# yahoo/TensorFlowOnSpark

Hardware: AMD Instinct MI355X
Metric: images/sec (whole node) ResNet-50 sync-SGD InputMode.SPARK (higher is better)
Workload: dtype bf16; 1 GPU; model=resnet50, global_batch=1024, per_gpu_batch=1024, parallelism=dp1

## Files before the change

### csrc/bindings.cpp

```cpp
#include <torch/extension.h>
#include <c10/hip/HIPStream.h>
#include <hip/hip_runtime.h>

extern "C" {
int tfosr_bn_fast_blocks(long, int, int, int);
void tfosr_bn_stats(const void*, int, int, float*, int, int, int, long, hipStream_t);
void tfosr_bn_finalize(const float*, int, const void*, int, int, long,
                       float*, float*, float*, float*,
                       long, int, float, float, hipStream_t);
void tfosr_bn_apply(const void*, const void*, void*, unsigned char*,
                    const float*, const float*,
                    const float*, const float*, int, int, int, long, int, long,
                    hipStream_t);
void tfosr_bn_bwd_stats(const void*, const void*, const void*,
                        const unsigned char*, void*,
                        const float*, const float*, float*, int, int, int,
                        int, int, int, long, hipStream_t);
void tfosr_bn_bwd_merge(const float*, int, float*, float*, int, hipStream_t);
void tfosr_bn_bwd_dx(const void*, const void*, const void*,
                     const unsigned char*, const float*,
                     const float*, const float*, const float*, const float*,
                     void*, int, int, int, long, int, long, hipStream_t);
int tfosr_xent_dense_grid(int, int, long, long, int, int);
void tfosr_xent_dense_fwd(int, const void*, const long*, float*, float*, float*,
                          int*, int, long, long, int, long, float, int,
                          hipStream_t);
void tfosr_xent_dense_finalize(const float*, const int*, int, int, float*, int*,
                               hipStream_t);
void tfosr_xent_dense_bwd(int, const void*, const float*, const long*,
                          const float*, const float*, const int*, int, void*,
                          int, long, long, int, long, float, int, hipStream_t);
void tfosr_nhwc_pack(const void*, void*, const float*, const float*, float, int,
                     int, long, int, long, hipStream_t);
void tfosr_sgd_step(float*, const float*, float*, float, float, float, int, long,
                    hipStream_t);
void tfosr_adam_step(float*, const float*, float*, float*, float, float, float,
                     float, float, int, int, long, hipStream_t);
void tfosr_gemm_bt(const void*, const void*, void*, int, int, int, int,
                   hipStream_t);
void tfosr_gemm_bt_acc(const void*, const void*, void*, int, int, int, int,
                       int, hipStream_t);
void tfosr_mfma_probe(const short*, const short*, float*, hipStream_t);
void tfosr_maxpool_fwd(const void*, void*, unsigned char*, int, int, int, int,
                       int, int, int, int, int, int, hipStream_t);
void tfosr_maxpool_bwd(const void*, const unsigned char*, void*, int, int, int,
                       int, int, int, int, int, int, int, hipStream_t);
void tfosr_conv3x3(const void*, const void*, const void*, void*, int, int, int,
                   int, int, int, int, int, int, int, hipStream_t);
void tfosr_conv_mfma(const void*, const void*, const void*, void*, int, int,
                     int, int, int, int, int, int, int, int, int, int, int,
                     int, int, hipStream_t);
void tfosr_conv_wrw(const void*, const void*, float*, int, int, int, int, int,
                    int, int, int, int, int, hipStream_t);
int tfosr_wrw2_split(int, int, long);
void tfosr_conv_wrw2(const void*, const void*, const void*, float*, float*,
                     int, int, int, int, int, int, int, int, int, int, int,
                     int, int, hipStream_t);
void tfosr_conv_stem(const void*, const void*, const void*, void*, int, int,
// ... 152 lines not shown
  int bf = dtype_flag(x);
  bn_check_like(dy, x, l.nhwc, false, "dy");
  bn_check_like(y, x, l.nhwc, true, "y");
  bn_check_channel_vec(w, x, l.C, "weight");
  bn_check_channel_vec(save_mean, x, l.C, "save_mean");
  bn_check_channel_vec(save_rstd, x, l.C, "save_rstd");
  dy = l.nhwc ? dy.contiguous(at::MemoryFormat::ChannelsLast) : dy.contiguous();
  auto opts = x.options().dtype(at::kFloat);
  long total = (long)l.N * l.HW * l.C;
  int nb = tfosr_bn_fast_blocks(total, l.C, bf, l.nhwc);
  auto ws = nb > 0 ? at::empty({(long)nb * 2 * l.C}, opts)
                   : at::zeros({2L * l.C}, opts);
  auto dg = at::empty({l.C}, opts);
  auto db = at::empty({l.C}, opts);
  auto dx = at::empty_like(x);
  at::Tensor gout;
  void* gout_ptr = nullptr;
  if (grad_res) {
    gout = at::empty_like(x);
    gout_ptr = gout.data_ptr();
  }
  auto s = cur_stream();
  const unsigned char* mask_ptr =
      mask.numel() ? mask.data_ptr<unsigned char>() : nullptr;
  TORCH_CHECK(!(relu && nb > 0) || mask_ptr != nullptr,
              "fast-path relu backward requires the forward bitmask");
  if (relu && nb > 0) {
    TORCH_CHECK(mask.device() == x.device() && mask.scalar_type() == at::kByte &&
                    mask.is_contiguous() && mask.numel() == total / (bf ? 8 : 4),
                "bn: mask must be the contiguous uint8 bitmask bn_fwd_train "
                "returned for this input");
  }
  tfosr_bn_bwd_stats(x.data_ptr(), dy.data_ptr(), y.data_ptr(), mask_ptr,
                     gout_ptr,
                     save_mean.data_ptr<float>(), save_rstd.data_ptr<float>(),
                     ws.data_ptr<float>(), nb, bf, l.nhwc,
                     relu, l.N, l.C, l.HW, s);
  tfosr_bn_bwd_merge(ws.data_ptr<float>(), nb, dg.data_ptr<float>(),
                     db.data_ptr<float>(), l.C, s);
  if (grad_res) {
    tfosr_bn_bwd_dx(x.data_ptr(), gout.data_ptr(), y.data_ptr(), nullptr,
                    save_mean.data_ptr<float>(), save_rstd.data_ptr<float>(),
                    w.data_ptr<float>(), dg.data_ptr<float>(), db.data_ptr<float>(),
                    dx.data_ptr(), bf, l.nhwc, 0, total, l.C, l.HW, s);
    return {dx, dg, db, gout};
  }
  tfosr_bn_bwd_dx(x.data_ptr(), dy.data_ptr(), y.data_ptr(), mask_ptr,
                  save_mean.data_ptr<float>(), save_rstd.data_ptr<float>(),
                  w.data_ptr<float>(), dg.data_ptr<float>(), db.data_ptr<float>(),
                  dx.data_ptr(), bf, l.nhwc, relu, total, l.C, l.HW, s);
  return {dx, dg, db};
}


enum { XENT_ROWS = 0, XENT_STRIDED = 1, XENT_TILE = 2 };
enum { XENT_NONE = 0, XENT_SUM = 1, XENT_MEAN = 2 };

struct XentLayout {
  int family;
  long P, S;
  int C;
};

XentLayout xent_layout(const at::Tensor& logits, const at::Tensor& target) {
  TORCH_CHECK(logits.is_cuda(), "xent: logits must be a GPU tensor");
  TORCH_CHECK(logits.scalar_type() == at::kFloat ||
                  logits.scalar_type() == at::kBFloat16,
              "xent: logits must be float32 or bfloat16");
  TORCH_CHECK(logits.dim() >= 2, "xent: logits must be (P, C) or (N, C, d1, ...)");
  TORCH_CHECK(target.device() == logits.device(),
              "xent: target must be on ", logits.device());
  TORCH_CHECK(target.scalar_type() == at::kLong, "xent: target must be int64");
  TORCH_CHECK(target.is_contiguous(), "xent: target must be contiguous");
  TORCH_CHECK(target.dim() == logits.dim() - 1 &&
                  target.size(0) == logits.size(0),
              "xent: target must have the logits' shape without the class dim");
  for (int64_t d = 2; d < logits.dim(); ++d)
    TORCH_CHECK(target.size(d - 1) == logits.size(d),
                "xent: target must have the logits' shape without the class dim");
  TORCH_CHECK(logits.size(1) >= 1 && logits.size(1) < (1L << 24),
              "xent: bad class count");
  XentLayout l;
  l.C = (int)logits.size(1);
  l.P = target.numel();
  l.S = 1;
  bool rows;
  if (logits.dim() == 2) {
    TORCH_CHECK(logits.is_contiguous(), "xent: 2-D logits must be contiguous");
    rows = true;
  } else if (logits.is_contiguous()) {
    rows = false;
    for (int64_t d = 2; d < logits.dim(); ++d) l.S *= logits.size(d);
  } else {
    TORCH_CHECK(logits.dim() == 4 &&
                    logits.is_contiguous(at::MemoryFormat::ChannelsLast),
                "xent: N-D logits must be contiguous or 4-D channels_last");
    rows = true;
  }
  l.family = rows ? (l.C >= 64 ? XENT_ROWS : XENT_TILE) : XENT_STRIDED;
  return l;
}

void xent_check_rowvec(const at::Tensor& t, const at::Tensor& logits, long P,
                       const char* name) {
  TORCH_CHECK(t.device() == logits.device() && t.scalar_type() == at::kFloat &&
                  t.is_contiguous() && t.numel() == P,
// ... 136 lines not shown
  TORCH_CHECK(p.scalar_type() == at::kFloat, "sgd_step expects fp32 params");
  tfosr_sgd_step(p.data_ptr<float>(), g.data_ptr<float>(), m.data_ptr<float>(),
                 (float)lr, (float)mu, (float)wd, nesterov, p.numel(),
                 cur_stream());
}

at::Tensor gemm_bt(at::Tensor a, at::Tensor b, bool out_bf16) {
  TORCH_CHECK(a.dim() == 2 && b.dim() == 2 && a.size(1) == b.size(1),
              "gemm_bt: A[M,K], B[N,K]");
  TORCH_CHECK(a.scalar_type() == at::kBFloat16 && b.scalar_type() == at::kBFloat16);
  int M = a.size(0), N = b.size(0), K = a.size(1);
  if (K % 32 != 0) {
    int Kp = (K + 31) / 32 * 32;
    auto ap = at::zeros({M, Kp}, a.options());
    auto bp = at::zeros({N, Kp}, b.options());
    ap.narrow(1, 0, K).copy_(a);
    bp.narrow(1, 0, K).copy_(b);
    a = ap; b = bp; K = Kp;
  }
  a = a.contiguous();
  b = b.contiguous();
  auto out = at::empty({M, N}, a.options().dtype(out_bf16 ? at::kBFloat16
                                                          : at::kFloat));
  tfosr_gemm_bt(a.data_ptr(), b.data_ptr(), out.data_ptr(), out_bf16, M, N, K,
                cur_stream());
  return out;
}

at::Tensor gemm_bf16(at::Tensor a, at::Tensor b) {
  return gemm_bt(a, b.t().contiguous(), false);
}

at::Tensor mfma_probe(at::Tensor a, at::Tensor b) {
  TORCH_CHECK(a.sizes() == at::IntArrayRef({64, 8}) &&
              b.sizes() == at::IntArrayRef({64, 8}));
  auto c = at::empty({64, 4}, a.options().dtype(at::kFloat));
  tfosr_mfma_probe(a.contiguous().data_ptr<short>(),
                   b.contiguous().data_ptr<short>(), c.data_ptr<float>(),
                   cur_stream());
  return c;
}

}

#define TFOSR_API_VERSION 6

static constexpr long kMaxTapReach = 1L << 20;

PYBIND11_MODULE(TORCH_EXTENSION_NAME, m) {
  m.def("api_version", []() { return TFOSR_API_VERSION; });
  m.def("bn_fwd_train", &bn_fwd_train);
  m.def("bn_fwd_eval", &bn_fwd_eval);
  m.def("bn_bwd", &bn_bwd);
  m.def("softmax_xent_fwd", &softmax_xent_fwd);
  m.def("softmax_xent_bwd", &softmax_xent_bwd);
  m.def("xent_dense_fwd", &xent_dense_fwd, py::arg("logits"), py::arg("target"),
        py::arg("ignore_index") = -100, py::arg("label_smoothing") = 0.0,
        py::arg("reduction") = 0, py::arg("max_grid") = 0);
  m.def("xent_dense_bwd", &xent_dense_bwd, py::arg("logits"), py::arg("lse"),
        py::arg("target"), py::arg("gout"), py::arg("nvalid") = py::none(),
        py::arg("ignore_index") = -100, py::arg("label_smoothing") = 0.0,
        py::arg("reduction") = 0, py::arg("max_grid") = 0);
  m.def("nhwc_pack", &nhwc_pack);
  m.def("sgd_step", &sgd_step);
  m.def("adam_step", [](at::Tensor p, at::Tensor g, at::Tensor m, at::Tensor v,
                        double lr, double b1, double b2, double eps, double wd,
                        long step, bool decoupled) {
    TORCH_CHECK(p.scalar_type() == at::kFloat);
    tfosr_adam_step(p.data_ptr<float>(), g.data_ptr<float>(),
                    m.data_ptr<float>(), v.data_ptr<float>(), lr, b1, b2, eps,
                    wd, (int)step, decoupled, p.numel(), cur_stream());
  });
  m.def("gemm_bt", &gemm_bt, py::arg("a"), py::arg("b"), py::arg("out_bf16") = false);
  m.def("gemm_bf16", &gemm_bf16);
  m.def("mfma_probe", &mfma_probe);
  m.def("maxpool_fwd", [](at::Tensor x, long K, long S, long P) {
    TORCH_CHECK(x.dim() == 4 && x.is_contiguous(at::MemoryFormat::ChannelsLast),
                "maxpool_fwd expects channels_last");
    int N = x.size(0), C = x.size(1), H = x.size(2), W = x.size(3);
    int OH = (H + 2 * P - K) / S + 1, OW = (W + 2 * P - K) / S + 1;
    TORCH_CHECK(C % (x.scalar_type() == at::kBFloat16 ? 8 : 4) == 0);
    auto y = at::empty({N, C, OH, OW}, x.options(),
                       at::MemoryFormat::ChannelsLast);
    auto idx = at::empty({N, OH, OW, C}, x.options().dtype(at::kByte));
    tfosr_maxpool_fwd(x.data_ptr(), y.data_ptr(), idx.data_ptr<unsigned char>(),
                      x.scalar_type() == at::kBFloat16, N, C, H, W, OH, OW,
                      K, S, P, cur_stream());
    return std::vector<at::Tensor>{y, idx};
  });
  m.def("conv3x3_fwd", [](at::Tensor x, at::Tensor w9, long Cout, long S,
                          long P) {
    TORCH_CHECK(x.dim() == 4 && x.is_contiguous(at::MemoryFormat::ChannelsLast),
                "conv3x3_fwd expects channels_last input");
    TORCH_CHECK(x.scalar_type() == at::kBFloat16 &&
                w9.scalar_type() == at::kBFloat16);
    int N = x.size(0), Cin = x.size(1), H = x.size(2), W = x.size(3);
    TORCH_CHECK(Cin % 32 == 0, "conv3x3 requires Cin % 32 == 0");
    TORCH_CHECK(w9.size(1) == 9 * Cin);
    int OH = (H + 2 * P - 3) / S + 1, OW = (W + 2 * P - 3) / S + 1;
    auto y = at::empty({N, Cout, OH, OW}, x.options(),
                       at::MemoryFormat::ChannelsLast);
    auto guard = at::zeros({64}, x.options());
    tfosr_conv3x3(x.data_ptr(), w9.contiguous().data_ptr(), guard.data_ptr(),
                  y.data_ptr(), 1, N, H, W, Cin, Cout, OH, OW,
                  S, P, cur_stream());
    return y;
// ... 230 lines not shown
```

### csrc/bn_relu.hip

```cpp
#include "tfosr_common.h"

typedef unsigned int u32;


template <typename T>
struct VecIO;

template <>
struct VecIO<bf16_t> {
  static constexpr int V = 8;
  using vec_t = s8v;
  __device__ static void load(const bf16_t* p, float* out) {
    vec_t v = *(const vec_t*)p;
    #pragma unroll
    for (int j = 0; j < 8; ++j) {
      union { short s; bf16_t b; } u;
      u.s = v[j];
      out[j] = (float)u.b;
    }
  }
  __device__ static void store(bf16_t* p, const float* in) {
    vec_t v;
    #pragma unroll
    for (int j = 0; j < 8; ++j) {
// ... 183 lines not shown
}

__global__ void bwd_stats_merge(const float* __restrict__ partials, int nblocks,
                                u32 C, float* __restrict__ dg,
                                float* __restrict__ db) {
  __shared__ float scratch[8];
  const u32 c = blockIdx.x;
  float sg = 0.f, sb = 0.f;
  for (int b = threadIdx.x; b < nblocks; b += blockDim.x) {
    sg += partials[(size_t)b * 2 * C + c];
    sb += partials[(size_t)b * 2 * C + C + c];
  }
  sg = block_sum<256>(sg, scratch);
  __syncthreads();
  sb = block_sum<256>(sb, scratch);
  if (threadIdx.x == 0) {
    dg[c] = sg;
    db[c] = sb;
  }
}

template <typename T, bool RELU>
__global__ void bwd_dx_fast(const T* __restrict__ x, const T* __restrict__ dy,
                            const unsigned char* __restrict__ mask,
                            T* __restrict__ dx,
                            const float* __restrict__ mean,
                            const float* __restrict__ rstd,
                            const float* __restrict__ w,
                            const float* __restrict__ dg,
                            const float* __restrict__ db,
                            u32 nvec, u32 C, float invM) {
  constexpr int V = VecIO<T>::V;
  const u32 c0 = channel_slot<V>(C);
  float sc[V], mu[V], rs[V], dgm[V], dbm[V], xv[V], dv[V];
  #pragma unroll
  for (int j = 0; j < V; ++j) {
    mu[j] = mean[c0 + j]; rs[j] = rstd[c0 + j];
    sc[j] = w[c0 + j] * rs[j];
    dgm[j] = dg[c0 + j] * invM;
    dbm[j] = db[c0 + j] * invM;
  }
  const u32 stride = gridDim.x * blockDim.x;
  for (u32 i = blockIdx.x * blockDim.x + threadIdx.x; i < nvec; i += stride) {
    VecIO<T>::load(x + (size_t)i * V, xv);
    VecIO<T>::load(dy + (size_t)i * V, dv);
    unsigned char m = RELU ? mask[i] : 0;
    #pragma unroll
    for (int j = 0; j < V; ++j) {
      float g = RELU ? (((m >> j) & 1) ? dv[j] : 0.f) : dv[j];
      float xhat = (xv[j] - mu[j]) * rs[j];
      dv[j] = sc[j] * (g - dbm[j] - xhat * dgm[j]);
    }
    VecIO<T>::store(dx + (size_t)i * V, dv);
  }
}


#define TFOSR_BN_CHUNK 4096

template <bool NHWC>
__device__ __forceinline__ long pixel_index(long m, int c, int C, long HW) {
  return NHWC ? m * C + c : ((m / HW) * C + c) * HW + m % HW;
}

static inline dim3 generic_red_grid(long M, int C) {
  long chunks = (M + TFOSR_BN_CHUNK - 1) / TFOSR_BN_CHUNK;
  if (chunks > 1024) chunks = 1024;
  return dim3((unsigned)C, (unsigned)(chunks > 0 ? chunks : 1));
}

template <typename T, bool NHWC>
__global__ void stats_generic(const T* __restrict__ x, float* __restrict__ ws,
                              long M, int C, long HW) {
  __shared__ float scratch[8];
  __shared__ float shift;
  const int c = blockIdx.x;
  if (threadIdx.x == 0)
    shift = channel_shift(x, c, C, HW, NHWC,
                          M < TFOSR_BN_SHIFT_PIXELS ? (int)M : TFOSR_BN_SHIFT_PIXELS);
  __syncthreads();
  const float k = shift;
  float s = 0.f, q = 0.f;
  for (long m0 = (long)blockIdx.y * TFOSR_BN_CHUNK; m0 < M;
       m0 += (long)gridDim.y * TFOSR_BN_CHUNK) {
    const long m1 = m0 + TFOSR_BN_CHUNK < M ? m0 + TFOSR_BN_CHUNK : M;
    for (long m = m0 + threadIdx.x; m < m1; m += blockDim.x) {
      float d = (float)x[pixel_index<NHWC>(m, c, C, HW)] - k;
      s += d;
      q += d * d;
    }
  }
  s = block_sum<256>(s, scratch);
  __syncthreads();
  q = block_sum<256>(q, scratch);
  if (threadIdx.x == 0) {
    atomicAdd(&ws[c], s);
    atomicAdd(&ws[C + c], q);
  }
}

template <typename T, bool NHWC, bool RELU, bool ADD>
__global__ void bn_apply_generic(const T* __restrict__ x, const T* __restrict__ res,
                                 T* __restrict__ y,
                                 const float* __restrict__ mean,
                                 const float* __restrict__ rstd,
                                 const float* __restrict__ w,
// ... 208 lines not shown
                   else { if (wg) BS_GEN(bf16_t, true, false, true); else BS_GEN(bf16_t, true, false, false); } }
    else { if (relu) { if (wg) BS_GEN(bf16_t, false, true, true); else BS_GEN(bf16_t, false, true, false); }
           else { if (wg) BS_GEN(bf16_t, false, false, true); else BS_GEN(bf16_t, false, false, false); } }
  } else {
    if (is_nhwc) { if (relu) { if (wg) BS_GEN(float, true, true, true); else BS_GEN(float, true, true, false); }
                   else { if (wg) BS_GEN(float, true, false, true); else BS_GEN(float, true, false, false); } }
    else { if (relu) { if (wg) BS_GEN(float, false, true, true); else BS_GEN(float, false, true, false); }
           else { if (wg) BS_GEN(float, false, false, true); else BS_GEN(float, false, false, false); } }
  }
#undef BS_GEN
}

void tfosr_bn_bwd_merge(const float* partials, int nb, float* dg, float* db,
                        int C, hipStream_t s) {
  hipLaunchKernelGGL(bwd_stats_merge, dim3(C), dim3(256), 0, s,
                     partials, nb > 0 ? nb : 1, (u32)C, dg, db);
}

void tfosr_bn_bwd_dx(const void* x, const void* dy, const void* y,
                     const unsigned char* mask,
                     const float* mean, const float* rstd, const float* w,
                     const float* dg, const float* db, void* dx, int is_bf16,
                     int is_nhwc, int relu, long total, int C, long HW,
                     hipStream_t s) {
  const float invM = 1.f / (float)(total / C);
  int vec = is_bf16 ? 8 : 4;
  if (fast_ok(is_nhwc, total, C, vec)) {
    u32 nvec = (u32)(total / vec);
    int grid = fast_grid(nvec, grid_quantum(C, vec));
#define DX_FAST(T, R) \
    hipLaunchKernelGGL((bwd_dx_fast<T, R>), dim3(grid), dim3(256), 0, s, \
                       (const T*)x, (const T*)dy, mask, (T*)dx, \
                       mean, rstd, w, dg, db, nvec, (u32)C, invM)
    if (is_bf16) { if (relu) DX_FAST(bf16_t, true); else DX_FAST(bf16_t, false); }
    else { if (relu) DX_FAST(float, true); else DX_FAST(float, false); }
#undef DX_FAST
    return;
  }
  int grid = tfosr_grid(total, 256);
#define DX_GEN(T, L, R) \
  hipLaunchKernelGGL((bwd_dx_generic<T, L, R>), dim3(grid), dim3(256), 0, s, \
                     (const T*)x, (const T*)dy, (const T*)y, (T*)dx, \
                     mean, rstd, w, dg, db, total, C, HW, invM)
  if (is_bf16) {
    if (is_nhwc) { if (relu) DX_GEN(bf16_t, true, true); else DX_GEN(bf16_t, true, false); }
    else { if (relu) DX_GEN(bf16_t, false, true); else DX_GEN(bf16_t, false, false); }
  } else {
    if (is_nhwc) { if (relu) DX_GEN(float, true, true); else DX_GEN(float, true, false); }
    else { if (relu) DX_GEN(float, false, true); else DX_GEN(float, false, false); }
  }
#undef DX_GEN
}

}
```

### tensorflowonspark_amd/ops/modules.py

```python

import torch
import torch.nn as nn
import torch.nn.functional as F

from . import get_ext




def _use_wrw2(k, cin, cout):
    import os
    mode = os.environ.get("TFOS_WRW", "auto")
    if mode == "mfma2":
        return True
    if mode in ("miopen", "mfma"):
        return False
    return k == 3 and cin <= 64 and cout <= 64



class _FusedBNFn(torch.autograd.Function):

    @staticmethod
    def forward(ctx, x, res, weight, bias, running_mean, running_var,
# ... 888 lines not shown
            bc1 = 1 - self.b1 ** self.step_count
            bc2 = 1 - self.b2 ** self.step_count
            upd = (m / bc1) / ((v / bc2).sqrt() + self.eps)
            if self.decoupled and self.weight_decay:
                upd = upd + self.weight_decay * pf
            pf.add_(upd, alpha=-self.lr)

    def zero_grad(self):
        self.engine.zero_grad()



class _BottleneckFn(torch.autograd.Function):

    @staticmethod
    def forward(ctx, x, w1, g1, b1, rm1, rv1, w2, g2, b2, rm2, rv2,
                w3, g3, b3, rm3, rv3, wd, gd, bd, rmd, rvd,
                stride, momentum, eps, packs=None):
        ext = get_ext(required=True)
        N, Cin, H, W = x.shape
        C1, C2, C3 = w1.shape[0], w2.shape[0], w3.shape[0]

        def as2d(t):
            return t.permute(0, 2, 3, 1).reshape(-1, t.shape[1])

        def as4d(t2, h, w):
            return t2.view(N, h, w, -1).permute(0, 3, 1, 2)

        if packs is not None:
            w1b = packs["w1b"].reshape(C1, Cin)
            w9 = packs["w9"].reshape(C2, 9 * C1)
            w3b = packs["w3b"].reshape(C3, C2)
        else:
            w1b = w1.view(C1, Cin).to(torch.bfloat16).contiguous()
            w9 = w2.permute(0, 2, 3, 1).reshape(C2, 9 * C1) \
                .to(torch.bfloat16).contiguous()
            w3b = w3.view(C3, C2).to(torch.bfloat16).contiguous()
        t1 = as4d(ext.gemm_bt(as2d(x), w1b, True), H, W)
        a1, m1, r1, k1 = ext.bn_fwd_train(t1, None, g1, b1, rm1, rv1,
                                          momentum, eps, True)
        t2 = ext.conv_mfma(a1, w9, C2, 3, 3, stride, 1, 1, -1, -1)
        a2, m2, r2, k2 = ext.bn_fwd_train(t2, None, g2, b2, rm2, rv2,
                                          momentum, eps, True)
        OH, OW = t2.shape[2], t2.shape[3]
        t3 = as4d(ext.gemm_bt(as2d(a2), w3b, True), OH, OW)

        if wd is not None:
            wdb = packs["wdb"].reshape(C3, Cin) if packs is not None \
                else wd.view(C3, Cin).to(torch.bfloat16).contiguous()
            if stride == 1:
                td = as4d(ext.gemm_bt(as2d(x), wdb, True), H, W)
            else:
                td = ext.conv_mfma(x, wdb, C3, 1, 1, stride, 0, 1, -1, -1)
            idn, md, rd, _kd = ext.bn_fwd_train(td, None, gd, bd, rmd, rvd,
                                                momentum, eps, False)
            opt = [td, idn, md, rd]
        else:
            idn = None
            opt = []
        res = idn if idn is not None else x
        y, m3, r3, k3 = ext.bn_fwd_train(t3, res, g3, b3, rm3, rv3,
                                         momentum, eps, True)

        ctx.save_for_backward(x, w1, g1, t1, a1, m1, r1, k1,
                              w2, g2, t2, a2, m2, r2, k2,
                              w3, g3, t3, m3, r3, k3, y, wd, gd, *opt)
        ctx.meta = (stride, wd is not None)
        ctx.packs = packs
        return y

    @staticmethod
    def backward(ctx, dy):
        ext = get_ext(required=True)
        (x, w1, g1, t1, a1, m1, r1, k1, w2, g2, t2, a2, m2, r2, k2,
         w3, g3, t3, m3, r3, k3, y, wd, gd, *opt) = ctx.saved_tensors
        stride, has_down = ctx.meta
        packs = ctx.packs
        N, Cin, H, W = x.shape
        C1, C2, C3 = w1.shape[0], w2.shape[0], w3.shape[0]
        OH, OW = t2.shape[2], t2.shape[3]
        dy = dy.contiguous(memory_format=torch.channels_last)
        if dy.dtype != torch.bfloat16:
            dy = dy.to(torch.bfloat16)

        def as2d(t):
            return t.permute(0, 2, 3, 1).reshape(-1, t.shape[1])

        def as4d(t2d, h, w):
            return t2d.view(N, h, w, -1).permute(0, 3, 1, 2)

        def cl(t):
            return t.contiguous(memory_format=torch.channels_last)

        dt3, dg3, db3, dres = ext.bn_bwd(t3, dy, y, k3, g3, m3, r3,
                                         True, True)
        dt3 = cl(dt3)

        def lib_wrw(dyt, xt, w4, s_, p_):
            w4 = w4.to(torch.bfloat16).contiguous(
                memory_format=torch.channels_last)
            _, dw, _ = torch.ops.aten.convolution_backward(
                dyt, xt, w4, None, [s_, s_], [p_, p_], [1, 1], False, [0, 0],
                1, [False, True, False])
            return dw

        w3bT = packs["w3bT"].reshape(C2, C3) if packs is not None \
            else w3.view(C3, C2).to(torch.bfloat16).t().contiguous()
        da2 = cl(as4d(ext.gemm_bt(as2d(dt3), w3bT, True), OH, OW))
        dw3 = ext.conv_wrw2(dt3, a2, 1, 1, 1, 0).view(C3, C2, 1, 1) \
            if _use_wrw2(1, C2, C3) \
            else lib_wrw(dt3, a2, w3.view(C3, C2, 1, 1), 1, 0)

        dt2, dg2, db2 = ext.bn_bwd(t2, da2, a2, k2, g2, m2, r2, True, False)
        dt2 = cl(dt2)

        if stride == 2:
            da1 = torch.empty(N, C1, H, W, device=x.device,
                              dtype=torch.bfloat16) \
                .contiguous(memory_format=torch.channels_last)
            if packs is not None:
                _conv_parity_packed(dt2, packs, "w9p", da1, 3, 1)
            else:
                wperm2 = w2.flip(2, 3).permute(1, 2, 3, 0) \
                    .to(torch.bfloat16).contiguous()
                _conv_parity(dt2, wperm2, da1, 3, 1)
        else:
            w9p = packs["w9p"].reshape(C1, 9 * C2) if packs is not None \
                else w2.flip(2, 3).permute(1, 2, 3, 0).reshape(C1, 9 * C2) \
                .to(torch.bfloat16).contiguous()
            da1 = ext.conv_mfma(dt2, w9p, C1, 3, 3, 1, 1, 1, H, W)
        if _use_wrw2(3, C1, C2):
            dw9 = ext.conv_wrw2(dt2, a1, 3, 3, stride, 1)
            dw2 = dw9.view(C2, 3, 3, C1).permute(0, 3, 1, 2).contiguous()
        else:
            dw2 = lib_wrw(dt2, a1, w2, stride, 1)

        dt1, dg1, db1 = ext.bn_bwd(t1, da1, a1, k1, g1, m1, r1, True, False)
        dt1 = cl(dt1)

        dw1 = ext.conv_wrw2(dt1, x, 1, 1, 1, 0).view(C1, Cin, 1, 1) \
            if _use_wrw2(1, Cin, C1) \
            else lib_wrw(dt1, x, w1.view(C1, Cin, 1, 1), 1, 0)

        w1bT = packs["w1bT"].reshape(Cin, C1) if packs is not None \
            else w1.view(C1, Cin).to(torch.bfloat16).t().contiguous()
        if has_down:
            td, idn, md, rd = opt
            dtd, dgd, dbd = ext.bn_bwd(td, dres, idn,
                                       torch.empty(0, dtype=torch.uint8,
                                                   device=td.device),
                                       gd, md, rd, False, False)
            dtd = cl(dtd)
            dwd = ext.conv_wrw2(dtd, x, 1, 1, stride, 0) \
                .view(C3, Cin, 1, 1) if _use_wrw2(1, Cin, C3) \
                else lib_wrw(dtd, x, wd.view(C3, Cin, 1, 1), stride, 0)
            dx2d = ext.gemm_bt(as2d(dt1), w1bT, True)
            dx = cl(as4d(dx2d, H, W))
            wdbT = packs["wdbT"].reshape(Cin, C3) if packs is not None \
                else wd.view(C3, Cin).to(torch.bfloat16).t().contiguous()
            if stride == 1:
                ext.gemm_bt_acc(as2d(dtd), wdbT, as2d(dx))
            else:
                ext.conv_par(dtd, wdbT, dx, [0], [0], 0, True)
            dwd = dwd.to(wd.dtype)
            dgd_, dbd_ = dgd, dbd
        else:
            dx = dres
            ext.gemm_bt_acc(as2d(dt1), w1bT, as2d(dx))
            dwd = dgd_ = dbd_ = None

        return (dx, dw1.to(w1.dtype), dg1, db1, None, None,
                dw2.to(w2.dtype), dg2, db2, None, None,
                dw3.to(w3.dtype), dg3, db3, None, None,
                dwd, dgd_, dbd_, None, None,
                None, None, None, None)



class _StemConvFn(torch.autograd.Function):

    @staticmethod
    def forward(ctx, x, weight, w224=None):
        ext = get_ext(required=True)
        N, _, H, W = x.shape
        Cout = weight.shape[0]
        x4 = torch.zeros(N, 4, H + 6, W + 6, dtype=torch.bfloat16,
                         device=x.device) \
            .contiguous(memory_format=torch.channels_last)
        x4[:, :3, 3:H + 3, 3:W + 3] = x
        if w224 is None:
            w224 = torch.zeros(Cout, 7, 8, 4, dtype=torch.bfloat16,
                               device=x.device)
            w224[:, :, :7, :3] = weight.permute(0, 2, 3, 1).to(torch.bfloat16)
        y = ext.conv_stem(x4, w224.reshape(Cout, 224).contiguous(), Cout)
        ctx.save_for_backward(x4, weight)
        return y

    @staticmethod
    def backward(ctx, dy):
        ext = get_ext(required=True)
        x4, weight = ctx.saved_tensors
        dy = dy.contiguous(memory_format=torch.channels_last)
        if dy.dtype != torch.bfloat16:
            dy = dy.to(torch.bfloat16)
# ... 101 lines not shown
```

Baseline: 9818 images/sec.

## Fuse downsample and main-branch BatchNorm into dual BN kernels for bottleneck blocks

For bottleneck blocks with a downsample branch, the two BatchNorms (bn3 and the downsample bn) are computed jointly. One apply kernel normalises both inputs, adds them, applies ReLU and writes the mask. In backward, a single stats pass and a single dx pass produce gradients for both branches. This avoids materialising the normalised identity tensor and cuts several full-tensor read/write passes and kernel launches. The cost is more live registers per thread in the dual kernels, and it adds an environment-variable switch plus a new bn_stage binding.

```diff
diff --git a/csrc/bindings.cpp b/csrc/bindings.cpp
--- a/csrc/bindings.cpp
+++ b/csrc/bindings.cpp
@@ -4,6 +4,21 @@
 
 extern "C" {
 int tfosr_bn_fast_blocks(long, int, int, int);
+void tfosr_bn_apply_dual(const void*, const void*, void*, unsigned char*,
+                         const float*, const float*, const float*, const float*,
+                         const float*, const float*, const float*, const float*,
+                         int, long, int, hipStream_t);
+void tfosr_bn_bwd_stats_dual(const void*, const void*, const void*,
+                             const unsigned char*, const float*, const float*,
+                             const float*, const float*, float*, int, int, long,
+                             int, hipStream_t);
+void tfosr_bn_bwd_merge_dual(const float*, int, float*, float*, float*, float*,
+                             int, hipStream_t);
+void tfosr_bn_bwd_dx_dual(const void*, const void*, const void*,
+                          const unsigned char*, void*, void*, const float*,
+                          const float*, const float*, const float*, const float*,
+                          const float*, const float*, const float*, const float*,
+                          int, long, int, hipStream_t);
 void tfosr_bn_stats(const void*, int, int, float*, int, int, int, long, hipStream_t);
 void tfosr_bn_finalize(const float*, int, const void*, int, int, long,
                        float*, float*, float*, float*,
@@ -262,6 +277,157 @@
   return {dx, dg, db};
 }
 
+bool bn_dual_eligible(const at::Tensor& xa, const at::Tensor& xb) {
+  if (!xa.is_cuda() || !xb.is_cuda() || xa.dim() != 4) return false;
+  if (xa.scalar_type() != at::kBFloat16 && xa.scalar_type() != at::kFloat)
+    return false;
+  if (xb.scalar_type() != xa.scalar_type() || xb.device() != xa.device() ||
+      xb.sizes() != xa.sizes())
+    return false;
+  if (!xa.is_contiguous(at::MemoryFormat::ChannelsLast) ||
+      !xb.is_contiguous(at::MemoryFormat::ChannelsLast))
+    return false;
+  return tfosr_bn_fast_blocks(xa.numel(), (int)xa.size(1),
+                              xa.scalar_type() == at::kBFloat16, 1) > 0;
+}
+
+std::vector<at::Tensor> bn_dual_fwd_train(
+    at::Tensor xa, at::Tensor xb, at::Tensor w_a, at::Tensor b_a,
+    at::Tensor rm_a, at::Tensor rv_a, at::Tensor w_b, at::Tensor b_b,
+    at::Tensor rm_b, at::Tensor rv_b, double momentum, double eps) {
+  TORCH_CHECK(bn_dual_eligible(xa, xb),
+              "bn_dual: needs two same-shape channels_last GPU tensors on the "
+              "NHWC fast path");
+  auto l = bn_layout(xa);
+  int bf = dtype_flag(xa);
+  const at::Tensor* vecs[] = {&w_a, &b_a, &rm_a, &rv_a, &w_b, &b_b, &rm_b, &rv_b};
+  for (auto* t : vecs) bn_check_channel_vec(*t, xa, l.C, "per-channel vector");
+  auto opts = xa.options().dtype(at::kFloat);
+  long M = (long)l.N * l.HW;
+  long total = M * l.C;
+  int nb = tfosr_bn_fast_blocks(total, l.C, bf, 1);
+  auto ws = at::empty({(long)nb * 2 * l.C}, opts);
+  auto mean_a = at::empty({l.C}, opts), rstd_a = at::empty({l.C}, opts);
+  auto mean_b = at::empty({l.C}, opts), rstd_b = at::empty({l.C}, opts);
+  auto y = at::empty_like(xa);
+  auto mask = at::empty({total / (bf ? 8 : 4)}, xa.options().dtype(at::kByte));
+  auto s = cur_stream();
+  auto f = [](at::Tensor& t) { return t.data_ptr<float>(); };
+  tfosr_bn_stats(xa.data_ptr(), bf, 1, f(ws), nb, l.N, l.C, l.HW, s);
+  tfosr_bn_finalize(f(ws), nb, xa.data_ptr(), bf, 1, l.HW, f(mean_a), f(rstd_a),
+                    f(rm_a), f(rv_a), M, l.C, (float)momentum, (float)eps, s);
+  tfosr_bn_stats(xb.data_ptr(), bf, 1, f(ws), nb, l.N, l.C, l.HW, s);
+  tfosr_bn_finalize(f(ws), nb, xb.data_ptr(), bf, 1, l.HW, f(mean_b), f(rstd_b),
+                    f(rm_b), f(rv_b), M, l.C, (float)momentum, (float)eps, s);
+  tfosr_bn_apply_dual(xa.data_ptr(), xb.data_ptr(), y.data_ptr(),
+                      mask.data_ptr<unsigned char>(), f(mean_a), f(rstd_a),
+                      f(w_a), f(b_a), f(mean_b), f(rstd_b), f(w_b), f(b_b), bf,
+                      total, l.C, s);
+  return {y, mean_a, rstd_a, mean_b, rstd_b, mask};
+}
+
+std::vector<at::Tensor> bn_dual_bwd(at::Tensor xa, at::Tensor xb, at::Tensor dy,
+                                    at::Tensor mask, at::Tensor w_a,
+                                    at::Tensor mean_a, at::Tensor rstd_a,
+                                    at::Tensor w_b, at::Tensor mean_b,
+                                    at::Tensor rstd_b) {
+  TORCH_CHECK(bn_dual_eligible(xa, xb),
+              "bn_dual: needs two same-shape channels_last GPU tensors on the "
+              "NHWC fast path");
+  auto l = bn_layout(xa);
+  int bf = dtype_flag(xa);
+  bn_check_like(dy, xa, true, false, "dy");
+  dy = dy.contiguous(at::MemoryFormat::ChannelsLast);
+  const at::Tensor* vecs[] = {&w_a, &mean_a, &rstd_a, &w_b, &mean_b, &rstd_b};
+  for (auto* t : vecs) bn_check_channel_vec(*t, xa, l.C, "per-channel vector");
+  long total = (long)l.N * l.HW * l.C;
+  TORCH_CHECK(mask.device() == xa.device() && mask.scalar_type() == at::kByte &&
+                  mask.is_contiguous() && mask.numel() == total / (bf ? 8 : 4),
+              "bn_dual: mask must be the contiguous uint8 bitmask "
+              "bn_dual_fwd_train returned for these inputs");
+  auto opts = xa.options().dtype(at::kFloat);
+  int nb = tfosr_bn_fast_blocks(total, l.C, bf, 1);
+  auto ws = at::empty({(long)nb * 3 * l.C}, opts);
+  auto dg_a = at::empty({l.C}, opts), dg_b = at::empty({l.C}, opts);
+  auto db_a = at::empty({l.C}, opts), db_b = at::empty({l.C}, opts);
+  auto dxa = at::empty_like(xa), dxb = at::empty_like(xb);
+  auto s = cur_stream();
+  auto f = [](at::Tensor& t) { return t.data_ptr<float>(); };
+  const unsigned char* mask_ptr = mask.data_ptr<unsigned char>();
+  tfosr_bn_bwd_stats_dual(xa.data_ptr(), xb.data_ptr(), dy.data_ptr(), mask_ptr,
+                          f(mean_a), f(rstd_a), f(mean_b), f(rstd_b), f(ws), nb,
+                          bf, total, l.C, s);
+  tfosr_bn_bwd_merge_dual(f(ws), nb, f(dg_a), f(dg_b), f(db_a), f(db_b), l.C, s);
+  tfosr_bn_bwd_dx_dual(xa.data_ptr(), xb.data_ptr(), dy.data_ptr(), mask_ptr,
+                       dxa.data_ptr(), dxb.data_ptr(), f(mean_a), f(rstd_a),
+                       f(w_a), f(dg_a), f(mean_b), f(rstd_b), f(w_b), f(dg_b),
+                       f(db_a), bf, total, l.C, s);
+  return {dxa, dxb, dg_a, dg_b, db_a, db_b};
+}
+
+void bn_stage(int family, at::Tensor x, c10::optional<at::Tensor> other,
+              c10::optional<at::Tensor> out, c10::optional<at::Tensor> mask,
+              at::Tensor ws, std::vector<at::Tensor> p, bool relu) {
+  auto l = bn_layout(x);
+  int bf = dtype_flag(x);
+  long total = (long)l.N * l.HW * l.C;
+  int nb = tfosr_bn_fast_blocks(total, l.C, bf, l.nhwc);
+  TORCH_CHECK(nb > 0, "bn_stage: shape is not on the NHWC fast path");
+  const size_t need[4] = {0, 4, 2, 5};
+  TORCH_CHECK(family >= 0 && family < 4, "bn_stage: family must be 0..3");
+  TORCH_CHECK(p.size() == need[family], "bn_stage: family ", family, " takes ",
+              need[family], " per-channel vectors");
+  for (auto& t : p) bn_check_channel_vec(t, x, l.C, "per-channel vector");
+  TORCH_CHECK(ws.device() == x.device() && ws.scalar_type() == at::kFloat &&
+                  ws.is_contiguous() && ws.numel() >= (long)nb * 2 * l.C,
+              "bn_stage: ws must hold bn_fast_blocks() * 2C floats");
+  const void* other_ptr = nullptr;
+  if (other.has_value()) {
+    bn_check_like(*other, x, l.nhwc, true, "other");
+    other_ptr = other->data_ptr();
+  }
+  void* out_ptr = nullptr;
+  if (out.has_value()) {
+    bn_check_like(*out, x, l.nhwc, true, "out");
+    out_ptr = out->data_ptr();
+  }
+  unsigned char* mask_ptr = nullptr;
+  if (mask.has_value()) {
+    TORCH_CHECK(mask->device() == x.device() && mask->scalar_type() == at::kByte &&
+                    mask->is_contiguous() && mask->numel() == total / (bf ? 8 : 4),
+                "bn_stage: mask must be a contiguous uint8 tensor, one byte "
+                "per 16 B vector");
+    mask_ptr = mask->data_ptr<unsigned char>();
+  }
+  if (family != 0 && family != 1)
+    TORCH_CHECK(other_ptr != nullptr, "bn_stage: dy is required");
+  if (family == 1 || family == 3)
+    TORCH_CHECK(out_ptr != nullptr, "bn_stage: out is required");
+  if (family >= 2)
+    TORCH_CHECK(!relu || mask_ptr != nullptr, "bn_stage: relu needs the mask");
+  auto f = [&](size_t i) { return p[i].data_ptr<float>(); };
+  auto s = cur_stream();
+  switch (family) {
+    case 0:
+      tfosr_bn_stats(x.data_ptr(), bf, 1, ws.data_ptr<float>(), nb, l.N, l.C,
+                     l.HW, s);
+      break;
+    case 1:
+      tfosr_bn_apply(x.data_ptr(), other_ptr, out_ptr, mask_ptr, f(0), f(1),
+                     f(2), f(3), bf, 1, relu, total, l.C, l.HW, s);
+      break;
+    case 2:
+      tfosr_bn_bwd_stats(x.data_ptr(), other_ptr, nullptr, mask_ptr, out_ptr,
+                         f(0), f(1), ws.data_ptr<float>(), nb, bf, 1, relu,
+                         l.N, l.C, l.HW, s);
+      break;
+    default:
+      tfosr_bn_bwd_dx(x.data_ptr(), other_ptr, nullptr, mask_ptr, f(0), f(1),
+                      f(2), f(3), f(4), out_ptr, bf, 1, relu, total, l.C, l.HW,
+                      s);
+  }
+}
+
 
 enum { XENT_ROWS = 0, XENT_STRIDED = 1, XENT_TILE = 2 };
 enum { XENT_NONE = 0, XENT_SUM = 1, XENT_MEAN = 2 };
@@ -504,6 +670,13 @@
   m.def("bn_fwd_train", &bn_fwd_train);
   m.def("bn_fwd_eval", &bn_fwd_eval);
   m.def("bn_bwd", &bn_bwd);
+  m.def("bn_dual_eligible", &bn_dual_eligible);
+  m.def("bn_dual_fwd_train", &bn_dual_fwd_train);
+  m.def("bn_dual_bwd", &bn_dual_bwd);
+  m.def("bn_fast_blocks", [](long total, int C, bool bf16, bool nhwc) {
+    return tfosr_bn_fast_blocks(total, C, bf16, nhwc);
+  });
+  m.def("bn_stage", &bn_stage);
   m.def("softmax_xent_fwd", &softmax_xent_fwd);
   m.def("softmax_xent_bwd", &softmax_xent_bwd);
   m.def("xent_dense_fwd", &xent_dense_fwd, py::arg("logits"), py::arg("target"),
diff --git a/csrc/bn_relu.hip b/csrc/bn_relu.hip
--- a/csrc/bn_relu.hip
+++ b/csrc/bn_relu.hip
@@ -259,6 +259,174 @@
       dv[j] = sc[j] * (g - dbm[j] - xhat * dgm[j]);
     }
     VecIO<T>::store(dx + (size_t)i * V, dv);
+  }
+}
+
+
+template <typename T>
+__global__ void bn_apply_dual_fast(const T* __restrict__ xa,
+                                   const T* __restrict__ xb, T* __restrict__ y,
+                                   unsigned char* __restrict__ mask,
+                                   const float* __restrict__ mean_a,
+                                   const float* __restrict__ rstd_a,
+                                   const float* __restrict__ w_a,
+                                   const float* __restrict__ b_a,
+                                   const float* __restrict__ mean_b,
+                                   const float* __restrict__ rstd_b,
+                                   const float* __restrict__ w_b,
+                                   const float* __restrict__ b_b,
+                                   u32 nvec, u32 C) {
+  constexpr int V = VecIO<T>::V;
+  const u32 c0 = channel_slot<V>(C);
+  float sca[V], mua[V], sha[V], scb[V], mub[V], shb[V], va[V], vb[V];
+  #pragma unroll
+  for (int j = 0; j < V; ++j) {
+    sca[j] = w_a[c0 + j] * rstd_a[c0 + j];
+    mua[j] = mean_a[c0 + j];
+    sha[j] = b_a[c0 + j];
+    scb[j] = w_b[c0 + j] * rstd_b[c0 + j];
+    mub[j] = mean_b[c0 + j];
+    shb[j] = b_b[c0 + j];
+  }
+  const u32 stride = gridDim.x * blockDim.x;
+  for (u32 i = blockIdx.x * blockDim.x + threadIdx.x; i < nvec; i += stride) {
+    VecIO<T>::load(xa + (size_t)i * V, va);
+    VecIO<T>::load(xb + (size_t)i * V, vb);
+    unsigned char m = 0;
+    #pragma unroll
+    for (int j = 0; j < V; ++j) {
+      float o = (va[j] - mua[j]) * sca[j] + sha[j];
+      o += (vb[j] - mub[j]) * scb[j] + shb[j];
+      if (o > 0.f) m |= (1u << j);
+      va[j] = fmaxf(o, 0.f);
+    }
+    VecIO<T>::store(y + (size_t)i * V, va);
+    mask[i] = m;
+  }
+}
+
+template <typename T>
+__global__ void bwd_stats_dual_fast(const T* __restrict__ xa,
+                                    const T* __restrict__ xb,
+                                    const T* __restrict__ dy,
+                                    const unsigned char* __restrict__ mask,
+                                    const float* __restrict__ mean_a,
+                                    const float* __restrict__ rstd_a,
+                                    const float* __restrict__ mean_b,
+                                    const float* __restrict__ rstd_b,
+                                    float* __restrict__ partials, u32 nvec,
+                                    u32 C) {
+  extern __shared__ float lds[];
+  constexpr int V = VecIO<T>::V;
+  const u32 c0 = channel_slot<V>(C);
+  for (u32 i = threadIdx.x; i < 3 * C; i += blockDim.x) lds[i] = 0.f;
+  __syncthreads();
+  float sga[V], sgb[V], sb[V], av[V], bv[V], dv[V];
+  float mua[V], rsa[V], mub[V], rsb[V];
+  #pragma unroll
+  for (int j = 0; j < V; ++j) {
+    sga[j] = 0.f; sgb[j] = 0.f; sb[j] = 0.f;
+    mua[j] = mean_a[c0 + j]; rsa[j] = rstd_a[c0 + j];
+    mub[j] = mean_b[c0 + j]; rsb[j] = rstd_b[c0 + j];
+  }
+  const u32 stride = gridDim.x * blockDim.x;
+  for (u32 i = blockIdx.x * blockDim.x + threadIdx.x; i < nvec; i += stride) {
+    VecIO<T>::load(xa + (size_t)i * V, av);
+    VecIO<T>::load(xb + (size_t)i * V, bv);
+    VecIO<T>::load(dy + (size_t)i * V, dv);
+    unsigned char m = mask[i];
+    #pragma unroll
+    for (int j = 0; j < V; ++j) {
+      float g = ((m >> j) & 1) ? dv[j] : 0.f;
+      sb[j] += g;
+      sga[j] += g * (av[j] - mua[j]) * rsa[j];
+      sgb[j] += g * (bv[j] - mub[j]) * rsb[j];
+    }
+  }
+  #pragma unroll
+  for (int j = 0; j < V; ++j) {
+    atomicAdd(&lds[c0 + j], sga[j]);
+    atomicAdd(&lds[C + c0 + j], sgb[j]);
+    atomicAdd(&lds[2 * C + c0 + j], sb[j]);
+  }
+  __syncthreads();
+  float* out = partials + (size_t)blockIdx.x * 3 * C;
+  for (u32 i = threadIdx.x; i < 3 * C; i += blockDim.x) out[i] = lds[i];
+}
+
+__global__ void bwd_stats_dual_merge(const float* __restrict__ partials,
+                                     int nblocks, u32 C,
+                                     float* __restrict__ dg_a,
+                                     float* __restrict__ dg_b,
+                                     float* __restrict__ db_a,
+                                     float* __restrict__ db_b) {
+  __shared__ float scratch[8];
+  const u32 c = blockIdx.x;
+  float sa = 0.f, sg = 0.f, sb = 0.f;
+  for (int b = threadIdx.x; b < nblocks; b += blockDim.x) {
+    sa += partials[(size_t)b * 3 * C + c];
+    sg += partials[(size_t)b * 3 * C + C + c];
+    sb += partials[(size_t)b * 3 * C + 2 * C + c];
+  }
+  sa = block_sum<256>(sa, scratch);
+  __syncthreads();
+  sg = block_sum<256>(sg, scratch);
+  __syncthreads();
+  sb = block_sum<256>(sb, scratch);
+  if (threadIdx.x == 0) {
+    dg_a[c] = sa;
+    dg_b[c] = sg;
+    db_a[c] = sb;
+    db_b[c] = sb;
+  }
+}
+
+template <typename T>
+__global__ void bwd_dx_dual_fast(const T* __restrict__ xa,
+                                 const T* __restrict__ xb,
+                                 const T* __restrict__ dy,
+                                 const unsigned char* __restrict__ mask,
+                                 T* __restrict__ dxa, T* __restrict__ dxb,
+                                 const float* __restrict__ mean_a,
+                                 const float* __restrict__ rstd_a,
+                                 const float* __restrict__ w_a,
+                                 const float* __restrict__ dg_a,
+                                 const float* __restrict__ mean_b,
+                                 const float* __restrict__ rstd_b,
+                                 const float* __restrict__ w_b,
+                                 const float* __restrict__ dg_b,
+                                 const float* __restrict__ db,
+                                 u32 nvec, u32 C, float invM) {
+  constexpr int V = VecIO<T>::V;
+  const u32 c0 = channel_slot<V>(C);
+  float sca[V], mua[V], rsa[V], dga[V], scb[V], mub[V], rsb[V], dgb[V], dbm[V];
+  float av[V], bv[V], dv[V];
+  #pragma unroll
+  for (int j = 0; j < V; ++j) {
+    mua[j] = mean_a[c0 + j]; rsa[j] = rstd_a[c0 + j];
+    sca[j] = w_a[c0 + j] * rsa[j];
+    dga[j] = dg_a[c0 + j] * invM;
+    mub[j] = mean_b[c0 + j]; rsb[j] = rstd_b[c0 + j];
+    scb[j] = w_b[c0 + j] * rsb[j];
+    dgb[j] = dg_b[c0 + j] * invM;
+    dbm[j] = db[c0 + j] * invM;
+  }
+  const u32 stride = gridDim.x * blockDim.x;
+  for (u32 i = blockIdx.x * blockDim.x + threadIdx.x; i < nvec; i += stride) {
+    VecIO<T>::load(xa + (size_t)i * V, av);
+    VecIO<T>::load(xb + (size_t)i * V, bv);
+    VecIO<T>::load(dy + (size_t)i * V, dv);
+    unsigned char m = mask[i];
+    #pragma unroll
+    for (int j = 0; j < V; ++j) {
+      float g = ((m >> j) & 1) ? dv[j] : 0.f;
+      float xhat_a = (av[j] - mua[j]) * rsa[j];
+      float xhat_b = (bv[j] - mub[j]) * rsb[j];
+      av[j] = sca[j] * (g - dbm[j] - xhat_a * dga[j]);
+      bv[j] = scb[j] * (g - dbm[j] - xhat_b * dgb[j]);
+    }
+    VecIO<T>::store(dxa + (size_t)i * V, av);
+    VecIO<T>::store(dxb + (size_t)i * V, bv);
   }
 }
 
@@ -573,4 +741,66 @@
 #undef DX_GEN
 }
 
-}
+
+void tfosr_bn_apply_dual(const void* xa, const void* xb, void* y,
+                         unsigned char* mask, const float* mean_a,
+                         const float* rstd_a, const float* w_a,
+                         const float* b_a, const float* mean_b,
+                         const float* rstd_b, const float* w_b,
+                         const float* b_b, int is_bf16, long total, int C,
+                         hipStream_t s) {
+  int vec = is_bf16 ? 8 : 4;
+  u32 nvec = (u32)(total / vec);
+  int grid = fast_grid(nvec, grid_quantum(C, vec));
+#define APPLY_DUAL(T) \
+  hipLaunchKernelGGL((bn_apply_dual_fast<T>), dim3(grid), dim3(256), 0, s, \
+                     (const T*)xa, (const T*)xb, (T*)y, mask, mean_a, rstd_a, \
+                     w_a, b_a, mean_b, rstd_b, w_b, b_b, nvec, (u32)C)
+  if (is_bf16) APPLY_DUAL(bf16_t); else APPLY_DUAL(float);
+#undef APPLY_DUAL
+}
+
+void tfosr_bn_bwd_stats_dual(const void* xa, const void* xb, const void* dy,
+                             const unsigned char* mask, const float* mean_a,
+                             const float* rstd_a, const float* mean_b,
+                             const float* rstd_b, float* partials, int nb,
+                             int is_bf16, long total, int C, hipStream_t s) {
+  int vec = is_bf16 ? 8 : 4;
+  u32 nvec = (u32)(total / vec);
+  size_t lds = 3 * (size_t)C * sizeof(float);
+#define BS_DUAL(T) \
+  hipLaunchKernelGGL((bwd_stats_dual_fast<T>), dim3(nb), dim3(256), lds, s, \
+                     (const T*)xa, (const T*)xb, (const T*)dy, mask, mean_a, \
+                     rstd_a, mean_b, rstd_b, partials, nvec, (u32)C)
+  if (is_bf16) BS_DUAL(bf16_t); else BS_DUAL(float);
+#undef BS_DUAL
+}
+
+void tfosr_bn_bwd_merge_dual(const float* partials, int nb, float* dg_a,
+                             float* dg_b, float* db_a, float* db_b, int C,
+                             hipStream_t s) {
+  hipLaunchKernelGGL(bwd_stats_dual_merge, dim3(C), dim3(256), 0, s,
+                     partials, nb, (u32)C, dg_a, dg_b, db_a, db_b);
+}
+
+void tfosr_bn_bwd_dx_dual(const void* xa, const void* xb, const void* dy,
+                          const unsigned char* mask, void* dxa, void* dxb,
+                          const float* mean_a, const float* rstd_a,
+                          const float* w_a, const float* dg_a,
+                          const float* mean_b, const float* rstd_b,
+                          const float* w_b, const float* dg_b, const float* db,
+                          int is_bf16, long total, int C, hipStream_t s) {
+  const float invM = 1.f / (float)(total / C);
+  int vec = is_bf16 ? 8 : 4;
+  u32 nvec = (u32)(total / vec);
+  int grid = fast_grid(nvec, grid_quantum(C, vec));
+#define DX_DUAL(T) \
+  hipLaunchKernelGGL((bwd_dx_dual_fast<T>), dim3(grid), dim3(256), 0, s, \
+                     (const T*)xa, (const T*)xb, (const T*)dy, mask, (T*)dxa, \
+                     (T*)dxb, mean_a, rstd_a, w_a, dg_a, mean_b, rstd_b, w_b, \
+                     dg_b, db, nvec, (u32)C, invM)
+  if (is_bf16) DX_DUAL(bf16_t); else DX_DUAL(float);
+#undef DX_DUAL
+}
+
+}
diff --git a/tensorflowonspark_amd/ops/modules.py b/tensorflowonspark_amd/ops/modules.py
--- a/tensorflowonspark_amd/ops/modules.py
+++ b/tensorflowonspark_amd/ops/modules.py
@@ -964,20 +964,29 @@
                 td = as4d(ext.gemm_bt(as2d(x), wdb, True), H, W)
             else:
                 td = ext.conv_mfma(x, wdb, C3, 1, 1, stride, 0, 1, -1, -1)
-            idn, md, rd, _kd = ext.bn_fwd_train(td, None, gd, bd, rmd, rvd,
-                                                momentum, eps, False)
-            opt = [td, idn, md, rd]
+            import os
+            dual = os.environ.get("TFOS_BN_DUAL", "on") != "off" \
+                and ext.bn_dual_eligible(t3, td)
+            if dual:
+                y, m3, r3, md, rd, k3 = ext.bn_dual_fwd_train(
+                    t3, td, g3, b3, rm3, rv3, gd, bd, rmd, rvd, momentum, eps)
+                opt = [td, md, rd]
+            else:
+                idn, md, rd, _kd = ext.bn_fwd_train(td, None, gd, bd, rmd,
+                                                    rvd, momentum, eps, False)
+                opt = [td, idn, md, rd]
         else:
-            idn = None
+            dual = False
+            idn = x
             opt = []
-        res = idn if idn is not None else x
-        y, m3, r3, k3 = ext.bn_fwd_train(t3, res, g3, b3, rm3, rv3,
-                                         momentum, eps, True)
+        if not dual:
+            y, m3, r3, k3 = ext.bn_fwd_train(t3, idn, g3, b3, rm3, rv3,
+                                             momentum, eps, True)
 
         ctx.save_for_backward(x, w1, g1, t1, a1, m1, r1, k1,
                               w2, g2, t2, a2, m2, r2, k2,
                               w3, g3, t3, m3, r3, k3, y, wd, gd, *opt)
-        ctx.meta = (stride, wd is not None)
+        ctx.meta = (stride, wd is not None, dual)
         ctx.packs = packs
         return y
 
@@ -986,7 +995,7 @@
         ext = get_ext(required=True)
         (x, w1, g1, t1, a1, m1, r1, k1, w2, g2, t2, a2, m2, r2, k2,
          w3, g3, t3, m3, r3, k3, y, wd, gd, *opt) = ctx.saved_tensors
-        stride, has_down = ctx.meta
+        stride, has_down, dual = ctx.meta
         packs = ctx.packs
         N, Cin, H, W = x.shape
         C1, C2, C3 = w1.shape[0], w2.shape[0], w3.shape[0]
@@ -1004,8 +1013,13 @@
         def cl(t):
             return t.contiguous(memory_format=torch.channels_last)
 
-        dt3, dg3, db3, dres = ext.bn_bwd(t3, dy, y, k3, g3, m3, r3,
-                                         True, True)
+        if dual:
+            td, md, rd = opt
+            dt3, dtd, dg3, dgd, db3, dbd = ext.bn_dual_bwd(
+                t3, td, dy, k3, g3, m3, r3, gd, md, rd)
+        else:
+            dt3, dg3, db3, dres = ext.bn_bwd(t3, dy, y, k3, g3, m3, r3,
+                                             True, True)
         dt3 = cl(dt3)
 
         def lib_wrw(dyt, xt, w4, s_, p_):
@@ -1057,11 +1071,12 @@
         w1bT = packs["w1bT"].reshape(Cin, C1) if packs is not None \
             else w1.view(C1, Cin).to(torch.bfloat16).t().contiguous()
         if has_down:
-            td, idn, md, rd = opt
-            dtd, dgd, dbd = ext.bn_bwd(td, dres, idn,
-                                       torch.empty(0, dtype=torch.uint8,
-                                                   device=td.device),
-                                       gd, md, rd, False, False)
+            if not dual:
+                td, idn, md, rd = opt
+                dtd, dgd, dbd = ext.bn_bwd(td, dres, idn,
+                                           torch.empty(0, dtype=torch.uint8,
+                                                       device=td.device),
+                                           gd, md, rd, False, False)
             dtd = cl(dtd)
             dwd = ext.conv_wrw2(dtd, x, 1, 1, stride, 0) \
                 .view(C3, Cin, 1, 1) if _use_wrw2(1, Cin, C3) \
```

After: 10050 images/sec (median of 6 runs). +2.3%, better.
